# RajaeeKh/TriNerfLet

Measured on NVIDIA B200. Metric: rays/sec per training step (fwd+bwd), higher is better.
Workload: dtype f16

## Files before the change

include/trinerflet_b200.h:

```cpp
#ifndef TRINERFLET_B200_H
#define TRINERFLET_B200_H

#include <stdint.h>

#ifdef __cplusplus
extern "C" {
#endif

#define TNL_ABI_VERSION 1
#define TNL_ERR_INVALID_ARGUMENT (-1)
#define TNL_ERR_UNSUPPORTED (-2)
#define TNL_ERR_WORKSPACE (-3)

typedef void* tnl_stream_t;

int tnl_abi_version(void);
const char* tnl_last_error(void);

int tnl_near_far_from_aabb(const float* rays_o, const float* rays_d, const float* aabb, uint32_t N,
                           float min_near, float* nears, float* fars, tnl_stream_t stream);
int tnl_sph_from_ray(const float* rays_o, const float* rays_d, float radius, uint32_t N, float* coords,
                     tnl_stream_t stream);
int tnl_morton3d(const int32_t* coords, uint32_t N, int32_t* indices, tnl_stream_t stream);
int tnl_morton3d_invert(const int32_t* indices, uint32_t N, int32_t* coords, tnl_stream_t stream);
// ... 72 lines not shown
typedef struct tnl_mlp_dims {
    uint32_t in_dim;
    uint32_t hidden;
    uint32_t hidden_c;
} tnl_mlp_dims;
size_t tnl_mlp_packed_bytes(const tnl_mlp_dims* dims);
int tnl_mlp_pack_weights(const tnl_mlp_dims* dims, const float* W1, const float* W2, const float* W3,
                         const float* W4, const float* W5, void* packed, tnl_stream_t stream);
int tnl_mlp_forward(const tnl_mlp_dims* dims, const void* packed, const void* feat, int feat_fp16, const float* dirs,
                    uint32_t M, const int32_t* n_valid, float* sigma, float* rgb, float* geo,
                    tnl_stream_t stream);
int tnl_mlp_backward(const tnl_mlp_dims* dims, const void* packed, const void* feat, int feat_fp16, const float* dirs,
                     uint32_t M, const int32_t* n_valid, const float* g_sigma, const float* g_rgb,
                     void* g_feat, float* g_W1, float* g_W2, float* g_W3, float* g_W4, float* g_W5,
                     tnl_stream_t stream);

int tnl_umma_probe(const void* A, int a_rows, int a_cols, const void* B, int b_rows, int b_cols, int a_mn, int b_mn,
                   int M, int N, int K, float* out, int ncols, tnl_stream_t stream);

int tnl_umma_bench(int a_rows, int b_rows, int a_mn, int b_mn, int M, int N, int K, int reps, long long* out2,
                   tnl_stream_t stream);
int tnl_umma_bench2(uint32_t a_lbo, uint32_t a_sbo, uint32_t a_step, uint32_t a_type, uint32_t b_lbo, uint32_t b_sbo,
                    uint32_t b_step, uint32_t b_type, int a_mn, int b_mn, int M, int N, int ksteps, int reps, long long* out2,
                    tnl_stream_t stream);
int tnl_mlp_tc_profile(unsigned long long* counters64);

int tnl_grad_nonfinite(const float* g, uint64_t n, float* found_inf, tnl_stream_t stream);
int tnl_adam_prepare(float* state3, const float* found_inf, float beta1, float beta2, tnl_stream_t stream);
int tnl_adam_step(float* p, const float* g, float* m, float* v, uint64_t n, const float* inv_scale, const float* found_inf,
                  const float* state3, float lr, float beta1, float beta2, float eps, float weight_decay, tnl_stream_t stream);
// ... 33 lines not shown
```

trinerflet_b200/_lib.py:

```python
import ctypes
import os

import torch

_HERE = os.path.dirname(os.path.abspath(__file__))
LIB_PATH = os.path.join(_HERE, "lib", "libtrinerflet_b200.so")

_c = ctypes
_vp, _u32, _f32, _int, _sz = _c.c_void_p, _c.c_uint32, _c.c_float, _c.c_int, _c.c_size_t


class MlpDims(ctypes.Structure):
    _fields_ = [("in_dim", _u32), ("hidden", _u32), ("hidden_c", _u32)]


_DP = ctypes.POINTER(MlpDims)

SIGNATURES = {
    "tnl_abi_version": (_int, []),
    "tnl_last_error": (_c.c_char_p, []),
    "tnl_near_far_from_aabb": (_int, [_vp, _vp, _vp, _u32, _f32, _vp, _vp, _vp]),
    "tnl_sph_from_ray": (_int, [_vp, _vp, _f32, _u32, _vp, _vp]),
    "tnl_morton3d": (_int, [_vp, _u32, _vp, _vp]),
    "tnl_morton3d_invert": (_int, [_vp, _u32, _vp, _vp]),
# ... 14 lines not shown
    "tnl_composite_rays_dev": (_int, [_vp, _u32, _f32, _vp, _vp, _vp, _vp, _vp, _vp, _vp, _vp, _vp]),
    "tnl_compact_alive_dev": (_int, [_vp, _u32, _vp, _vp, _vp, _sz, _vp]),
    "tnl_sh_encode_forward": (_int, [_vp, _vp, _u32, _u32, _vp]),
    "tnl_idwt_level_forward": (_int, [_vp, _vp, _vp, _u32, _u32, _vp, _vp]),
    "tnl_idwt_level_backward": (_int, [_vp, _vp, _vp, _u32, _u32, _vp, _vp, _f32, _u32, _u32, _vp]),
    "tnl_sample_planes_forward": (_int, [_vp, _vp, _u32, _u32, _u32, _f32, _int, _vp, _vp, _vp, _int, _vp]),
    "tnl_sample_planes_backward": (_int, [_vp, _int, _vp, _u32, _u32, _u32, _f32, _int, _vp, _vp, _vp, _vp]),
    "tnl_sample_planes_backward_plane": (_int, [_vp, _int, _vp, _u32, _u32, _u32, _f32, _int, _vp, _vp, _vp, _u32, _vp]),
    "tnl_sample_planes_backward_coords": (_int, [_vp, _vp, _vp, _u32, _u32, _u32, _f32, _int, _vp, _vp]),
    "tnl_cell_sort_workspace": (_sz, [_u32, _u32]),
    "tnl_cell_sort": (_int, [_vp, _u32, _vp, _f32, _u32, _vp, _vp, _sz, _vp]),
    "tnl_mlp_packed_bytes": (_sz, [_DP]),
    "tnl_mlp_pack_weights": (_int, [_DP, _vp, _vp, _vp, _vp, _vp, _vp, _vp]),
    "tnl_mlp_forward": (_int, [_DP, _vp, _vp, _int, _vp, _u32, _vp, _vp, _vp, _vp, _vp]),
    "tnl_mlp_backward": (_int, [_DP, _vp, _vp, _int, _vp, _u32, _vp, _vp, _vp, _vp, _vp, _vp, _vp, _vp, _vp, _vp]),
    "tnl_idwt_level_forward_sparse": (_int, [_vp, _vp, _vp, _u32, _u32, _vp, _vp, _vp, _vp, _u32, _u32, _u32, _vp]),
    "tnl_idwt_level_backward_sparse": (_int, [_vp, _vp, _vp, _u32, _u32, _vp, _vp, _f32, _vp, _vp, _vp, _u32, _u32, _u32, _vp, _vp]),
    "tnl_tiles_zero": (_int, [_vp, _vp, _vp, _u32, _u32, _u32, _u32, _vp]),
    "tnl_mlp_tc_profile": (_int, [_vp]),
    "tnl_umma_bench": (_int, [_int] * 8 + [_vp, _vp]),
    "tnl_umma_bench2": (_int, [_u32] * 8 + [_int] * 6 + [_vp, _vp]),
    "tnl_umma_probe": (_int, [_vp, _int, _int, _vp, _int, _int, _int, _int, _int, _int, _int, _vp, _int, _vp]),
    "tnl_mark_dirty_tiles": (_int, [_vp, _u32, _u32, _f32, _u32, _u32, _u32, _vp, _vp]),
    "tnl_tiles_pack": (_int, [_vp, _vp, _u32, _u32, _u32, _u32, _vp, _int, _vp]),
    "tnl_tiles_unpack": (_int, [_vp, _vp, _u32, _u32, _u32, _u32, _f32, _int, _vp, _vp]),
    "tnl_tiles_allreduce": (_int, [_vp, _vp, _vp, _vp, _u32, _u32, _u32, _u32, _u32, _u32, _f32, _vp]),
    "tnl_flat_allreduce": (_int, [_vp, _vp, _u32, _u32, _u32, _f32, _vp]),
    "tnl_grad_nonfinite": (_int, [_vp, ctypes.c_uint64, _vp, _vp]),
    "tnl_adam_prepare": (_int, [_vp, _vp, _f32, _f32, _vp]),
    "tnl_adam_step": (_int, [_vp, _vp, _vp, _vp, ctypes.c_uint64, _vp, _vp, _vp, _f32, _f32, _f32, _f32, _f32, _vp]),
# ... 87 lines not shown
```

trinerflet_b200/csrc/mlp.cu:

```cuda
#include "common.cuh"
#include "mlp_math.cuh"
#include "mlp_tc.cuh"
#include <stdlib.h>

namespace tnl {

struct MlpLayout {
    int K1, H, HC;
    int F1, F2, F3, F4, F5;
    int B1, B2, B3, B4, B5;
    int total;
};

__host__ __device__ constexpr MlpLayout make_layout(int K1, int H, int HC) {
    MlpLayout L{};
    L.K1 = K1; L.H = H; L.HC = HC;
    L.F1 = 0;
    L.F2 = L.F1 + (K1 / 16) * (H / 8) * 64;
    L.F3 = L.F2 + (H / 16) * 2 * 64;
    L.F4 = L.F3 + 2 * (HC / 8) * 64;
    L.F5 = L.F4 + (HC / 16) * (HC / 8) * 64;
    L.B5 = L.F5 + (HC / 16) * 1 * 64;
    L.B4 = L.B5 + 1 * (HC / 8) * 64;
    L.B3 = L.B4 + (HC / 16) * (HC / 8) * 64;
// ... 547 lines not shown

static bool dims_supported(const tnl_mlp_dims* d) {
    if (!d) return false;
    const bool k_ok = d->in_dim == 48 || d->in_dim == 96 || d->in_dim == 144;
    const bool h_ok = (d->hidden == 64 && d->hidden_c == 64) || (d->hidden == 128 && d->hidden_c == 128);
    return k_ok && h_ok;
}

static size_t legacy_packed_bytes(const tnl_mlp_dims* d) {
    const size_t b = sizeof(uint32_t) * (size_t)make_layout((int)d->in_dim, (int)d->hidden, (int)d->hidden_c).total;
    return (b + 255) & ~(size_t)255;
}
static bool use_tc(const tnl_mlp_dims* d, int feat_fp16) {
    static const bool legacy = getenv("TNL_MLP_LEGACY") != nullptr;
    return !legacy && feat_fp16 && mlp_tc_supported(d->in_dim, d->hidden, d->hidden_c);
}

#define TNL_MLP_DISPATCH(DIMS, CALL)                                                        \
    do {                                                                                    \
        const uint32_t k_ = (DIMS)->in_dim, h_ = (DIMS)->hidden;                            \
        if (k_ == 48 && h_ == 64) { CALL(48, 64, 64); }                                     \
        else if (k_ == 96 && h_ == 64) { CALL(96, 64, 64); }                                \
        else if (k_ == 144 && h_ == 64) { CALL(144, 64, 64); }                              \
        else if (k_ == 48 && h_ == 128) { CALL(48, 128, 128); }                             \
        else if (k_ == 96 && h_ == 128) { CALL(96, 128, 128); }                             \
        else { CALL(144, 128, 128); }                                                       \
    } while (0)

extern "C" {

// ... 104 lines not shown
```

trinerflet_b200/csrc/mlp_tc.cu:

```cuda
#include "common.cuh"
#include "mlp_math.cuh"
#include "mlp_tc.cuh"
#include "mlp_tc_util.cuh"
#include "umma.cuh"
#include <stdlib.h>

namespace tnl {
using namespace umma;

template <int K1>
struct TcW {
    static constexpr uint32_t W1 = 0;
    static constexpr uint32_t W2 = W1 + tile_bytes(64, K1);
    static constexpr uint32_t W3 = W2 + tile_bytes(16, 64);
    static constexpr uint32_t W4 = W3 + tile_bytes(64, 32);
    static constexpr uint32_t W5 = W4 + tile_bytes(64, 64);
    static constexpr uint32_t END = W5 + tile_bytes(16, 64);
};

__global__ void k_mlp_tc_pack(int K1, int H, const float* __restrict__ W1, const float* __restrict__ W2, const float* __restrict__ W3,
                              const float* __restrict__ W4, const float* __restrict__ W5, uint8_t* __restrict__ out) {
    const uint32_t n1 = H * K1, n2 = 16 * H, n3 = H * 32, n4 = H * H, n5 = 16 * H;
    uint32_t i = blockIdx.x * blockDim.x + threadIdx.x;
    uint32_t base = 0, R, Cc;
// ... 154 lines not shown
    static constexpr uint32_t H4 = H3 + tile_bytes(128, 64);
    static constexpr uint32_t D5 = H4 + tile_bytes(128, 64);
    static constexpr uint32_t SUB = D5 + tile_bytes(128, 16);
    static constexpr uint32_t SUB0 = TcW<K1>::END;
    static constexpr uint32_t BAR = SUB0 + 2 * SUB;
    static constexpr uint32_t TOTAL = BAR + 48;
};

__device__ __forceinline__ bool m64_row_of_lane(uint32_t warp, uint32_t lane, uint32_t& row) {
    row = warp * 16 + lane;
    return lane < 16;
}

constexpr int kBwdStages = 10;

template <int K1>
__global__ void __launch_bounds__(544, 1)
k_mlp_tc_bwd(const uint8_t* __restrict__ wpk, const __half* __restrict__ feat, const float* __restrict__ dirs, uint32_t M,
             const int32_t* __restrict__ n_valid_ptr, const float* __restrict__ g_sigma, const float* __restrict__ g_rgb,
             __half* __restrict__ g_feat, float* __restrict__ gW1, float* __restrict__ gW2, float* __restrict__ gW3,
             float* __restrict__ gW4, float* __restrict__ gW5, unsigned long long* __restrict__ dbg) {
    using W = TcW<K1>;
    using S = TcBwdSmem<K1>;
    constexpr uint32_t CW = K1 < 64 ? 64 : K1;
    constexpr uint32_t TM_C = 0, TM_W1 = 2 * CW, TM_W4 = TM_W1 + K1, TM_W3 = TM_W4 + 64, TM_W2 = TM_W3 + 32, TM_W5 = TM_W2 + 16;
    constexpr uint32_t TM_COLS = 512;
    static_assert(TM_W5 + 16 <= TM_COLS, "TMEM column budget");
    extern __shared__ __align__(128) uint8_t smem[];
    const uint32_t tid = threadIdx.x, warp = tid >> 5, lane = tid & 31;
    uint64_t* ready = reinterpret_cast<uint64_t*>(smem + S::BAR);
    uint64_t* done = reinterpret_cast<uint64_t*>(smem + S::BAR + 16);
    uint32_t* tslot = reinterpret_cast<uint32_t*>(smem + S::BAR + 32);
    for (uint32_t i = tid * 16; i < W::END; i += 544 * 16) *reinterpret_cast<uint4*>(smem + i) = __ldg(reinterpret_cast<const uint4*>(wpk + i));
    if (tid == 0) {
        mbar_init(&ready[0], 256); mbar_init(&ready[1], 256);
        mbar_init(&done[0], 1); mbar_init(&done[1], 1);
// ... 92 lines not shown
        float a[32];                                                                                                    \
        tmem_load_row<32>(trow + hf * 32u, a);                                                                          \
        _Pragma("unroll") for (int kc = 0; kc < 4; ++kc)                                                                \
            *reinterpret_cast<uint4*>(sub + (TILE) + ((hf * 4u + kc) * 128u + t) * 16u) = pack8<true>(a + 8 * kc);     \
    }
#define TNL_EPI_MASK(TILE)                                                                                              \
    {                                                                                                                   \
        float a[32];                                                                                                    \
        tmem_load_row<32>(trow + hf * 32u, a);                                                                          \
        _Pragma("unroll") for (int kc = 0; kc < 4; ++kc) {                                                              \
            uint4* q = reinterpret_cast<uint4*>(sub + (TILE) + ((hf * 4u + kc) * 128u + t) * 16u);                      \
            *q = mask8(pack8<false>(a + 8 * kc), *q);                                                                   \
        }                                                                                                               \
    }
        uint4 x[XH];
        {
            const uint32_t p0 = (2 * blockIdx.x + g) * 128 + t;
            const uint4* src = reinterpret_cast<const uint4*>(feat + (size_t)p0 * K1) + hf * XH;
#pragma unroll
            for (int kc = 0; kc < XH; ++kc) x[kc] = (my_pairs > 0 && p0 < nvalid) ? __ldg(src + kc) : make_uint4(0u, 0u, 0u, 0u);
        }
        for (uint32_t it = 0; it < my_pairs; ++it) {
            const uint32_t tile = 2 * (blockIdx.x + it * gridDim.x) + g;
            const uint32_t p = tile * 128 + t;
            const bool v = p < nvalid;
#pragma unroll
            for (int kc = 0; kc < XH; ++kc) *reinterpret_cast<uint4*>(sub + S::X + ((hf * XH + kc) * 128 + t) * 16) = x[kc];
            float d[3] = {0.f, 0.f, 0.f}, gr[3] = {0.f, 0.f, 0.f}, gs = 0.f;
            if (v && hf == 0) {
#pragma unroll
                for (int j = 0; j < 3; ++j) { d[j] = __ldg(dirs + 3 * (size_t)p + j); gr[j] = __ldg(g_rgb + 3 * (size_t)p + j); }
                gs = __ldg(g_sigma + p);
            }
            TNL_HANDOFF();
            {
                const uint32_t pn = (2 * (blockIdx.x + (it + 1) * gridDim.x) + g) * 128 + t;
                const uint4* src = reinterpret_cast<const uint4*>(feat + (size_t)pn * K1) + hf * XH;
                const bool vn = (it + 1 < my_pairs) && pn < nvalid;
#pragma unroll
                for (int kc = 0; kc < XH; ++kc) x[kc] = vn ? __ldg(src + kc) : make_uint4(0u, 0u, 0u, 0u);
            }
            TNL_EPI_RELU(S::H1);
            TNL_HANDOFF();
            float logit = 0.f;
            if (hf == 0) {
                float h2[16];
                tmem_load_row<16>(trow, h2);
#pragma unroll
                for (int j = 0; j < 16; ++j) h2[j] = r16(h2[j]);
                logit = h2[0];
                float in3[32];
                {
                    float sh[16];
// ... 19 lines not shown
#pragma unroll
                for (int j = 0; j < 3; ++j) {
                    const float sg = r16(sigmoidf_(r16(o[j])));
                    d5[j] = v ? r16(gr[j]) * sg * (1.f - sg) : 0.f;
                }
#pragma unroll
                for (int j = 3; j < 8; ++j) d5[j] = 0.f;
                *reinterpret_cast<uint4*>(sub + S::D5 + (0 * 128 + t) * 16) = pack8<false>(d5);
                *reinterpret_cast<uint4*>(sub + S::D5 + (1 * 128 + t) * 16) = make_uint4(0u, 0u, 0u, 0u);
            }
            TNL_HANDOFF();
            TNL_EPI_MASK(S::H4);
            TNL_HANDOFF();
            TNL_EPI_MASK(S::H3);
            TNL_HANDOFF();
            if (hf == 0) {
                float a[16];
                tmem_load_row<16>(trow, a);
                float dh2[16];
                dh2[0] = gs * expf(fminf(fmaxf(logit, -15.f), 15.f));
#pragma unroll
                for (int j = 0; j < 15; ++j) dh2[1 + j] = a[j];
                *reinterpret_cast<uint4*>(sub + S::I3 + (0 * 128 + t) * 16) = pack8<false>(dh2);
                *reinterpret_cast<uint4*>(sub + S::I3 + (1 * 128 + t) * 16) = pack8<false>(dh2 + 8);
            }
            TNL_HANDOFF();
            TNL_EPI_MASK(S::H1);
            TNL_HANDOFF();
            {
                float a[KH];
                tmem_load_row<KH>(trow + hf * KH, a);
                if (g_feat && p < M) {
                    uint4* dst = reinterpret_cast<uint4*>(g_feat + (size_t)p * K1 + hf * KH);
#pragma unroll
                    for (int kc = 0; kc < KH / 8; ++kc) dst[kc] = v ? pack8<false>(a + 8 * kc) : make_uint4(0u, 0u, 0u, 0u);
                }
            }
        }
#undef TNL_HANDOFF
#undef TNL_EPI_RELU
#undef TNL_EPI_MASK
    }
    fence_before_sync();
    __syncthreads();
// ... 185 lines not shown
                                                              n_valid, sigma, rgb, geo);
    else
        k_mlp_tc_fwd<K1, false><<<blocks, 128, S::TOTAL, s>>>(static_cast<const uint8_t*>(wpk), static_cast<const __half*>(feat), dirs, M,
                                                               n_valid, sigma, rgb, geo);
}

void mlp_tc_forward(uint32_t in_dim, uint32_t hidden, const void* wpk, const void* feat, const float* dirs, uint32_t M,
                    const int32_t* n_valid, float* sigma, float* rgb, float* geo, cudaStream_t s) {
    if (hidden == 128) { mlp_tc128_forward(in_dim, wpk, feat, dirs, M, n_valid, sigma, rgb, geo, s); return; }
    if (in_dim == 48) launch_fwd<48>(wpk, feat, dirs, M, n_valid, sigma, rgb, geo, s);
    else launch_fwd<96>(wpk, feat, dirs, M, n_valid, sigma, rgb, geo, s);
}

static unsigned long long* g_tc_dbg = nullptr;

template <int K1>
static void launch_bwd(const void* wpk, const void* feat, const float* dirs, uint32_t M, const int32_t* n_valid, const float* g_sigma,
                       const float* g_rgb, void* g_feat, float* gW1, float* gW2, float* gW3, float* gW4, float* gW5, cudaStream_t s) {
    using S = TcBwdSmem<K1>;
    cudaFuncSetAttribute(k_mlp_tc_bwd<K1>, cudaFuncAttributeMaxDynamicSharedMemorySize, (int)S::TOTAL);
    const uint32_t blocks = min(ceil_div(M, 256u), (uint32_t)kNumSM);
    k_mlp_tc_bwd<K1><<<blocks, 544, S::TOTAL, s>>>(static_cast<const uint8_t*>(wpk), static_cast<const __half*>(feat), dirs, M, n_valid,
                                                   g_sigma, g_rgb, static_cast<__half*>(g_feat), gW1, gW2, gW3, gW4, gW5, g_tc_dbg);
}

void mlp_tc_backward(uint32_t in_dim, uint32_t hidden, const void* wpk, const void* feat, const float* dirs, uint32_t M,
                     const int32_t* n_valid, const float* g_sigma, const float* g_rgb, void* g_feat, float* gW1, float* gW2, float* gW3,
                     float* gW4, float* gW5, cudaStream_t s) {
    if (hidden == 128) { mlp_tc128_backward(in_dim, wpk, feat, dirs, M, n_valid, g_sigma, g_rgb, g_feat, gW1, gW2, gW3, gW4, gW5, s); return; }
    if (in_dim == 48) launch_bwd<48>(wpk, feat, dirs, M, n_valid, g_sigma, g_rgb, g_feat, gW1, gW2, gW3, gW4, gW5, s);
    else launch_bwd<96>(wpk, feat, dirs, M, n_valid, g_sigma, g_rgb, g_feat, gW1, gW2, gW3, gW4, gW5, s);
}

}

using namespace tnl;

extern "C" int tnl_mlp_tc_profile(unsigned long long* counters64) {
    g_tc_dbg = counters64;
    return 0;
}

extern "C" int tnl_umma_bench(int a_rows, int b_rows, int a_mn, int b_mn, int M, int N, int K, int reps, long long* out2,
                              tnl_stream_t stream) {
    TNL_ARG_CHECK(out2, "null pointer");
    static bool attr = false;
    if (!attr) {
        cudaFuncSetAttribute(k_umma_bench, cudaFuncAttributeMaxDynamicSharedMemorySize, 160 * 1024);
        attr = true;
    }
    k_umma_bench<<<1, 128, 160 * 1024, reinterpret_cast<cudaStream_t>(stream)>>>(a_rows, b_rows, a_mn, b_mn, M, N, K, reps, out2);
    return finish_launch("umma_bench");
}

extern "C" int tnl_umma_bench2(uint32_t a_lbo, uint32_t a_sbo, uint32_t a_step, uint32_t a_type, uint32_t b_lbo, uint32_t b_sbo,
// ... 31 lines not shown
```

trinerflet_b200/csrc/mlp_tc.cuh:

```cuda
#pragma once
#include <cuda_runtime.h>
#include <stddef.h>
#include <stdint.h>

namespace tnl {

bool mlp_tc_supported(uint32_t in_dim, uint32_t hidden, uint32_t hidden_c);
size_t mlp_tc_packed_bytes(uint32_t in_dim, uint32_t hidden);
void mlp_tc_pack(uint32_t in_dim, uint32_t hidden, const float* W1, const float* W2, const float* W3, const float* W4, const float* W5,
                 void* out, cudaStream_t s);
void mlp_tc_forward(uint32_t in_dim, uint32_t hidden, const void* wpk, const void* feat, const float* dirs, uint32_t M,
                    const int32_t* n_valid, float* sigma, float* rgb, float* geo, cudaStream_t s);
void mlp_tc_backward(uint32_t in_dim, uint32_t hidden, const void* wpk, const void* feat, const float* dirs, uint32_t M,
                     const int32_t* n_valid, const float* g_sigma, const float* g_rgb, void* g_feat, float* gW1, float* gW2, float* gW3,
                     float* gW4, float* gW5, cudaStream_t s);
void mlp_tc128_forward(uint32_t in_dim, const void* wpk, const void* feat, const float* dirs, uint32_t M, const int32_t* n_valid,
                       float* sigma, float* rgb, float* geo, cudaStream_t s);
void mlp_tc128_backward(uint32_t in_dim, const void* wpk, const void* feat, const float* dirs, uint32_t M, const int32_t* n_valid,
                        const float* g_sigma, const float* g_rgb, void* g_feat, float* gW1, float* gW2, float* gW3, float* gW4, float* gW5,
                        cudaStream_t s);

}
```

trinerflet_b200/csrc/sample_coords.cuh:

```cuda
#pragma once
#include "common.cuh"

namespace tnl {

struct Tap {
    int x0, y0;
    float nw, ne, sw, se;
    bool x1ok, y1ok;
};

__device__ __forceinline__ float to_pixel(float g, int R) {
    float v = ((g + 1.0f) * 0.5f) * (float)(R - 1);
    return fminf((float)(R - 1), fmaxf(v, 0.0f));
}

__device__ __forceinline__ float to_pixel_grad(float g, int R, float& dg) {
    const float hi = (float)(R - 1);
    const float v = ((g + 1.0f) * 0.5f) * hi;
    if (!(v > 0.0f)) { dg = 0.0f; return 0.0f; }
    if (v >= hi) { dg = 0.0f; return hi; }
    dg = 0.5f * hi;
    return v;
}

// ... 1 lines not shown
    const float ix = to_pixel(gx, R), iy = to_pixel(gy, R);
    const float fx = floorf(ix), fy = floorf(iy);
    Tap t;
    t.x0 = (int)fx;
    t.y0 = (int)fy;
    const float ex = fx + 1.0f, ey = fy + 1.0f;
    t.nw = (ex - ix) * (ey - iy);
    t.ne = (ix - fx) * (ey - iy);
    t.sw = (ex - ix) * (iy - fy);
    t.se = (ix - fx) * (iy - fy);
    t.x1ok = t.x0 + 1 <= R - 1;
    t.y1ok = t.y0 + 1 <= R - 1;
    return t;
}

__device__ __forceinline__ float axis_coord(const float* __restrict__ xyz, uint32_t m, int a, float inv_bound, int fp16_coords) {
    float g = __fmul_rn(__ldg(xyz + 3 * (size_t)m + a), inv_bound);
    if (fp16_coords) g = __half2float(__float2half_rn(g));
    return g;
}

__device__ __forceinline__ void plane_coords(const float* __restrict__ xyz, uint32_t m, int p, float inv_bound,
                                             int fp16_coords, float& gx, float& gy) {
    const int a = (p == 2) ? 1 : 0;
    const int b = (p == 1) ? 1 : 2;
    gx = axis_coord(xyz, m, a, inv_bound, fp16_coords);
    gy = axis_coord(xyz, m, b, inv_bound, fp16_coords);
}

__device__ __forceinline__ uint2 pack4h(float4 v) {
    const __half2 a = __floats2half2_rn(v.x, v.y), b = __floats2half2_rn(v.z, v.w);
    return make_uint2(*reinterpret_cast<const uint32_t*>(&a), *reinterpret_cast<const uint32_t*>(&b));
}
__device__ __forceinline__ float4 unpack4h(uint2 u) {
// ... 6 lines not shown
```

trinerflet_b200/network.py:

```python
import ctypes

import torch
import torch.nn as nn
import torch.nn.functional as F
from torch.autograd import Function

from . import _lib
from ._lib import MlpDims, call, ptr, stream
from .activation import trunc_exp
from .encoding import get_encoder
from .renderer import NeRFRenderer


def fused_dims_supported(in_dim, hidden, hidden_color):
    return in_dim in (48, 96, 144) and hidden == hidden_color and hidden in (64, 128)


def pack_mlp_weights(dims, weights):
    lib = _lib.load()
    nbytes = lib.tnl_mlp_packed_bytes(ctypes.byref(dims))
    if nbytes == 0:
        raise RuntimeError("trinerflet_b200: unsupported MLP dimensions for the fused kernel")
    packed = torch.empty(nbytes, dtype=torch.uint8, device=weights[0].device)
    ws = [w.detach().contiguous().float() for w in weights]
    call("tnl_mlp_pack_weights", ctypes.byref(dims), *[ptr(w) for w in ws], ptr(packed), stream())
    return packed
# ... 1 lines not shown

_warned_library_path = False


def _warn_library_path(net, x):
    global _warned_library_path
    if not _warned_library_path and x.is_cuda:
        import warnings
        why = ("MLP dimensions outside the fused kernels" if not fused_dims_supported(net.in_dim, net.hidden_dim, net.hidden_dim_color)
               else "no CUDA fp16 autocast is active")
        warnings.warn(f"trinerflet_b200.NeRFNetwork: {why}; the sigma/color heads run as plain torch ops (library GEMMs), not the "
                      "fused sm_100a kernels. Wrap the call in torch.autocast('cuda', dtype=torch.float16) as the reference's --fp16 does.")
        _warned_library_path = True


class _FieldMLP(Function):

    @staticmethod
    def forward(ctx, feat, dirs, n_valid, W1, W2, W3, W4, W5):
        feat = feat.contiguous()
        ctx.in_dtype = feat.dtype
        if W1.shape[0] != 64:
            feat = feat.half()
        elif feat.dtype != torch.float16:
            feat = feat.float()
        fh = int(feat.dtype == torch.float16)
        dirs = dirs.detach().contiguous().float()
        M = feat.shape[0]
        dims = MlpDims(W1.shape[1], W1.shape[0], W4.shape[0])
        packed = pack_mlp_weights(dims, (W1, W2, W3, W4, W5))
        sigma = torch.empty(M, device=feat.device, dtype=torch.float32)
        rgb = torch.empty(M, 3, device=feat.device, dtype=torch.float32)
        call("tnl_mlp_forward", ctypes.byref(dims), ptr(packed), ptr(feat), fh, ptr(dirs), M, ptr(n_valid), ptr(sigma),
             ptr(rgb), None, stream())
        ctx.save_for_backward(feat, dirs, packed, n_valid if n_valid is not None else torch.empty(0))
        ctx.dims = (dims.in_dim, dims.hidden, dims.hidden_c, n_valid is not None)
        ctx.wshapes = [tuple(w.shape) for w in (W1, W2, W3, W4, W5)]
        return sigma, rgb

    @staticmethod
    def backward(ctx, g_sigma, g_rgb):
        feat, dirs, packed, n_valid = ctx.saved_tensors
        in_dim, hidden, hidden_c, has_nv = ctx.dims
        dims = MlpDims(in_dim, hidden, hidden_c)
        M = feat.shape[0]
        g_sigma = g_sigma.contiguous().float()
        g_rgb = g_rgb.contiguous().float()
        g_feat = torch.empty_like(feat)
        gW = [torch.zeros(s, device=feat.device, dtype=torch.float32) for s in ctx.wshapes]
        call("tnl_mlp_backward", ctypes.byref(dims), ptr(packed), ptr(feat), int(feat.dtype == torch.float16), ptr(dirs), M,
             ptr(n_valid) if has_nv else None, ptr(g_sigma), ptr(g_rgb), ptr(g_feat), *[ptr(g) for g in gW], stream())
        if g_feat.dtype != ctx.in_dtype:
            g_feat = g_feat.to(ctx.in_dtype)
        return (g_feat, None, None, *gW)


class _DensityMLP(Function):

    @staticmethod
    def forward(ctx, feat, W1, W2, W3, W4, W5):
        feat = feat.contiguous()
        if feat.dtype != torch.float16:
            feat = feat.float()
        M = feat.shape[0]
        dims = MlpDims(W1.shape[1], W1.shape[0], W4.shape[0])
        packed = pack_mlp_weights(dims, (W1, W2, W3, W4, W5))
        sigma = torch.empty(M, device=feat.device, dtype=torch.float32)
        geo = torch.empty(M, 15, device=feat.device, dtype=torch.float32)
        call("tnl_mlp_forward", ctypes.byref(dims), ptr(packed), ptr(feat), int(feat.dtype == torch.float16), None, M, None,
# ... 36 lines not shown
        return (self.sigma_net[0].weight, self.sigma_net[1].weight, self.color_net[0].weight, self.color_net[1].weight,
                self.color_net[2].weight)

    def _fused(self):
        return (torch.is_autocast_enabled("cuda") and torch.get_autocast_dtype("cuda") == torch.float16
                and fused_dims_supported(self.in_dim, self.hidden_dim, self.hidden_dim_color))

    spatial_sort_min_points = 1 << 18

    def forward(self, x, d, n_valid=None):
        perm = None
        if x.is_cuda and x.shape[0] >= self.spatial_sort_min_points and torch.is_grad_enabled():
            from .triplane_encoder import cell_sort
            perm = cell_sort(x, self.bound, n_valid, 64)
        fused = self._fused()
        feat = self.encoder(x, bound=self.bound, n_valid=n_valid, perm=perm, half_out=fused)
        if fused:
            return _FieldMLP.apply(feat, d, n_valid, *self._weights())
        _warn_library_path(self, x)
        h = F.relu(self.sigma_net[0](feat))
        h = self.sigma_net[1](h)
        sigma = trunc_exp(h[..., 0])
        geo_feat = h[..., 1:]
        h = torch.cat([self.encoder_dir(d), geo_feat], dim=-1)
        h = F.relu(self.color_net[0](h))
        h = F.relu(self.color_net[1](h))
        color = torch.sigmoid(self.color_net[2](h))
        return sigma, color

    def density(self, x):
# ... 31 lines not shown
```

trinerflet_b200/triplane_encoder.py:

```python
import math

import numpy as np
import torch
import torch.nn as nn
from torch.autograd import Function

from ._lib import call, ptr, stream

PAD_DICT = {'bior6.8': 4}


def get_levels(upscale_factor):
    wavelet_levels = math.log2(upscale_factor)
    if abs(wavelet_levels - round(wavelet_levels)) > 1e-5:
        raise ValueError('Unsupported res. should be 2^')
    return round(wavelet_levels)


def cl_empty_planes(C, n, device=None, dtype=torch.float32, zero=False):
    f = torch.zeros if zero else torch.empty
    return f(3, n, n, C, device=device, dtype=dtype).permute(0, 3, 1, 2)


def cl_empty_coefs(C, n, device=None, dtype=torch.float32, zero=False):
# ... 166 lines not shown
            p.grad = g


def build_planes_with_abs(planes_features, coefs, plan=None):
    return _BuildPlanes.apply(planes_features, plan, *coefs)


def build_planes(planes_features, coefs, plan=None):
    return _BuildPlanes.apply(planes_features, plan, *coefs)[0]


def _inv_bound(bound):
    return float(np.float32(1.0) / np.float32(bound))


class _SamplePlanes(Function):
    @staticmethod
    def forward(ctx, planes, coords, bound, fp16_coords, n_valid, perm=None, half_out=False, grad_buf=None):
        _require_cuda_f32(planes, "planes")
        ctx.grad_buf = grad_buf
        planes_cl = to_cl_planes(planes.detach())
        coords = coords.detach().contiguous().float()
        M = coords.shape[0]
        C, R = planes.shape[1], planes.shape[2]
        feat = torch.empty(M, 3 * C, device=planes.device, dtype=torch.float16 if half_out else torch.float32)
        inv = _inv_bound(bound)
        call("tnl_sample_planes_forward", ptr(planes_cl), ptr(coords), M, R, C, inv, int(bool(fp16_coords)),
             ptr(n_valid), ptr(perm), ptr(feat), int(bool(half_out)), stream())
        ctx.save_for_backward(coords, n_valid if n_valid is not None else torch.empty(0),
                              perm if perm is not None else torch.empty(0))
        ctx.meta = (M, R, C, inv, int(bool(fp16_coords)), n_valid is not None, perm is not None, bool(half_out))
        return feat

    @staticmethod
    def backward(ctx, g_feat):
        coords, n_valid, perm = ctx.saved_tensors
        M, R, C, inv, fp16_coords, has_nv, has_perm, half = ctx.meta
        g_feat = g_feat.contiguous().half() if half else g_feat.contiguous().float()
        external = False
        if ctx.grad_buf is not None:
            g_planes, ready, external, plane_hook = ctx.grad_buf
            ctx.grad_buf = None
            torch.cuda.current_stream().wait_event(ready)
        else:
            g_planes = cl_empty_planes(C, R, device=g_feat.device, zero=True)
            plane_hook = None
        if plane_hook is not None and C in (16, 32, 48):
            for p in range(3):
                call("tnl_sample_planes_backward_plane", ptr(g_feat), int(half), ptr(coords), M, R, C, inv, fp16_coords,
                     ptr(n_valid) if has_nv else None, ptr(perm) if has_perm else None, ptr(g_planes), p, stream())
                plane_hook(p)
        else:
            call("tnl_sample_planes_backward", ptr(g_feat), int(half), ptr(coords), M, R, C, inv, fp16_coords,
                 ptr(n_valid) if has_nv else None, ptr(perm) if has_perm else None, ptr(g_planes), stream())
        if external:
            return None, None, None, None, None, None, None, None
        return g_planes, None, None, None, None, None, None, None


def cell_sort(coords, bound, n_valid=None, G=64):
    from . import _lib
# ... 222 lines not shown
    def get_grid_features(self, grid_res, plane_features=None, grid=None):
        if grid is None:
            axis = torch.arange(grid_res)
            gx, gy, gz = torch.meshgrid(axis, axis, axis, indexing='xy')
            grid = torch.stack([gx, gy, gz], dim=-1) / (grid_res - 1)
        assert grid.max() <= 1 and grid.min() >= 0
        grid = 2 * self.lbound * grid - self.lbound
        grid = grid[..., [2, 0, 1]]
        if plane_features is None:
            plane_features = self.get_planes(2 * grid_res)
        grid = grid.to(device=plane_features.device, dtype=plane_features.dtype)
        shape = grid.shape
        feats = self.sample_from_planes(grid.reshape(-1, 3), plane_features=plane_features)
        return self.lbound, feats.reshape(*shape[:-1], -1), grid

    def forward(self, coordinates, bound, n_valid=None, perm=None, half_out=False):
        planes = self.get_planes()
        gbuf = self._join_prefetch()
        if gbuf is not None and not torch.is_grad_enabled():
            gbuf = None
        return sample_planes(planes, coordinates, bound, n_valid=n_valid, perm=perm, half_out=half_out, grad_buf=gbuf)

    def _load_from_state_dict(self, state_dict, prefix, *args, **kwargs):
        super()._load_from_state_dict(state_dict, prefix, *args, **kwargs)
        self.last_used_planes = None
```

Baseline: 11.54 million.

## Fuse triplane gradient scatter into tcgen05 MLP backward kernel

Adds a SCATTER variant of the tcgen05 MLP backward kernel. Instead of writing g_feat to global memory and running a separate sample-planes backward kernel, it stages the input-feature gradient in shared memory and scatters it with bilinear weights into the plane gradients using vector red.add atomics. A new autograd Function fuses plane sampling and the MLP for the 64-wide heads when a cell-sort permutation exists, reading rows through perm. This removes the g_feat round trip and one kernel launch. The cost is more register and shared-memory pressure and atomic work inside the pipelined MLP kernel, which could stall its tensor-core stages.

```diff
diff --git a/include/trinerflet_b200.h b/include/trinerflet_b200.h
--- a/include/trinerflet_b200.h
+++ b/include/trinerflet_b200.h
@@ -110,6 +110,10 @@
                      uint32_t M, const int32_t* n_valid, const float* g_sigma, const float* g_rgb,
                      void* g_feat, float* g_W1, float* g_W2, float* g_W3, float* g_W4, float* g_W5,
                      tnl_stream_t stream);
+int tnl_mlp_backward_scatter(const tnl_mlp_dims* dims, const void* packed, const void* feat, const float* dirs, uint32_t M,
+                             const int32_t* n_valid, const int32_t* perm, const float* g_sigma, const float* g_rgb,
+                             const float* xyz, uint32_t R, uint32_t C, float inv_bound, int fp16_coords, float* g_planes,
+                             float* g_W1, float* g_W2, float* g_W3, float* g_W4, float* g_W5, tnl_stream_t stream);
 
 int tnl_umma_probe(const void* A, int a_rows, int a_cols, const void* B, int b_rows, int b_cols, int a_mn, int b_mn,
                    int M, int N, int K, float* out, int ncols, tnl_stream_t stream);
diff --git a/profiles/prof_bwd_kernels.py b/profiles/prof_bwd_kernels.py
--- /dev/null
+++ b/profiles/prof_bwd_kernels.py
@@ -0,0 +1,41 @@
+import json
+import os
+import sys
+
+sys.path.insert(0, os.path.dirname(os.path.dirname(os.path.abspath(__file__))))
+import torch
+from torch.profiler import ProfilerActivity, profile
+
+from trinerflet_b200 import scene, trainer
+from trinerflet_b200.network import NeRFNetwork
+
+name = os.environ.get("TNL_CONFIG", "base_light")
+cfg = scene.CONFIGS[name]
+steps = int(os.environ.get("TNL_STEPS", "10"))
+net = NeRFNetwork(bound=1.5, cuda_ray=True, density_thresh=10, min_near=0.2, triplane_channels=cfg["C"],
+                  triplane_resolution=cfg["R"], triplane_wavelet_levels=cfg["S"], hidden_dim=cfg["hidden"],
+                  hidden_dim_color=cfg["hidden"]).cuda()
+scene.init_model_(net, 0)
+scene.install_ball_occupancy(net, 0.75)
+ts = trainer.TrainStep(net, trainer.default_opt(), None)
+sc = scene.make_scene()
+g = torch.Generator().manual_seed(0)
+batches = [tuple(t.cuda() for t in scene.sample_batch(sc, cfg["rays"], g)) for _ in range(steps + 3)]
+ts.forward_backward(*batches[0], update_grid=False)
+net.mean_count = int(net.step_counter[0, 0].item())
+net.local_step = 0
+for b in batches[1:3]:
+    net.zero_grad(set_to_none=True)
+    ts.forward_backward(*b, update_grid=False)
+torch.cuda.synchronize()
+with profile(activities=[ProfilerActivity.CUDA]) as prof:
+    for b in batches[3:]:
+        net.zero_grad(set_to_none=True)
+        ts.forward_backward(*b, update_grid=False)
+    torch.cuda.synchronize()
+per = {}
+for ev in prof.key_averages():
+    if "k_mlp_tc_bwd" in ev.key or "k_sample_bwd4" in ev.key:
+        per[ev.key] = round(ev.device_time_total / 1e3 / steps, 4)
+print(json.dumps({"config": name, "samples": net.mean_count, "steps": steps, "device": torch.cuda.get_device_name(0),
+                  "ms_per_step": per, "sum_ms_per_step": round(sum(per.values()), 4)}))
diff --git a/trinerflet_b200/_lib.py b/trinerflet_b200/_lib.py
--- a/trinerflet_b200/_lib.py
+++ b/trinerflet_b200/_lib.py
@@ -52,6 +52,8 @@
     "tnl_mlp_pack_weights": (_int, [_DP, _vp, _vp, _vp, _vp, _vp, _vp, _vp]),
     "tnl_mlp_forward": (_int, [_DP, _vp, _vp, _int, _vp, _u32, _vp, _vp, _vp, _vp, _vp]),
     "tnl_mlp_backward": (_int, [_DP, _vp, _vp, _int, _vp, _u32, _vp, _vp, _vp, _vp, _vp, _vp, _vp, _vp, _vp, _vp]),
+    "tnl_mlp_backward_scatter": (_int, [_DP, _vp, _vp, _vp, _u32, _vp, _vp, _vp, _vp, _vp, _u32, _u32, _f32, _int, _vp, _vp, _vp,
+                                        _vp, _vp, _vp, _vp]),
     "tnl_idwt_level_forward_sparse": (_int, [_vp, _vp, _vp, _u32, _u32, _vp, _vp, _vp, _vp, _u32, _u32, _u32, _vp]),
     "tnl_idwt_level_backward_sparse": (_int, [_vp, _vp, _vp, _u32, _u32, _vp, _vp, _f32, _vp, _vp, _vp, _u32, _u32, _u32, _vp, _vp]),
     "tnl_tiles_zero": (_int, [_vp, _vp, _vp, _u32, _u32, _u32, _u32, _vp]),
diff --git a/trinerflet_b200/csrc/mlp.cu b/trinerflet_b200/csrc/mlp.cu
--- a/trinerflet_b200/csrc/mlp.cu
+++ b/trinerflet_b200/csrc/mlp.cu
@@ -585,6 +585,11 @@
 static bool use_tc(const tnl_mlp_dims* d, int feat_fp16) {
     static const bool legacy = getenv("TNL_MLP_LEGACY") != nullptr;
     return !legacy && feat_fp16 && mlp_tc_supported(d->in_dim, d->hidden, d->hidden_c);
+}
+
+namespace tnl {
+size_t mlp_tc_packed_offset(const tnl_mlp_dims* d) { return legacy_packed_bytes(d); }
+bool mlp_tc_selected(const tnl_mlp_dims* d) { return dims_supported(d) && use_tc(d, 1); }
 }
 
 #define TNL_MLP_DISPATCH(DIMS, CALL)                                                        \
diff --git a/trinerflet_b200/csrc/mlp_tc.cu b/trinerflet_b200/csrc/mlp_tc.cu
--- a/trinerflet_b200/csrc/mlp_tc.cu
+++ b/trinerflet_b200/csrc/mlp_tc.cu
@@ -2,6 +2,7 @@
 #include "mlp_math.cuh"
 #include "mlp_tc.cuh"
 #include "mlp_tc_util.cuh"
+#include "sample_coords.cuh"
 #include "umma.cuh"
 #include <stdlib.h>
 
@@ -192,12 +193,27 @@
 
 constexpr int kBwdStages = 10;
 
-template <int K1>
+struct PlaneScatter {
+    const int32_t* perm;
+    const float* xyz;
+    float* g_planes;
+    int R;
+    float inv_bound;
+    int fp16_coords;
+};
+
+__device__ __forceinline__ void red_add_v4(float* addr, float4 v, float w) {
+    asm volatile("red.global.add.v4.f32 [%0], {%1, %2, %3, %4};\n" ::"l"(addr), "f"(v.x * w), "f"(v.y * w), "f"(v.z * w),
+                 "f"(v.w * w)
+                 : "memory");
+}
+
+template <int K1, bool SCATTER>
 __global__ void __launch_bounds__(544, 1)
 k_mlp_tc_bwd(const uint8_t* __restrict__ wpk, const __half* __restrict__ feat, const float* __restrict__ dirs, uint32_t M,
              const int32_t* __restrict__ n_valid_ptr, const float* __restrict__ g_sigma, const float* __restrict__ g_rgb,
              __half* __restrict__ g_feat, float* __restrict__ gW1, float* __restrict__ gW2, float* __restrict__ gW3,
-             float* __restrict__ gW4, float* __restrict__ gW5, unsigned long long* __restrict__ dbg) {
+             float* __restrict__ gW4, float* __restrict__ gW5, unsigned long long* __restrict__ dbg, const PlaneScatter sc) {
     using W = TcW<K1>;
     using S = TcBwdSmem<K1>;
     constexpr uint32_t CW = K1 < 64 ? 64 : K1;
@@ -320,29 +336,34 @@
         }                                                                                                               \
     }
         uint4 x[XH];
+        uint32_t mx;
         {
             const uint32_t p0 = (2 * blockIdx.x + g) * 128 + t;
-            const uint4* src = reinterpret_cast<const uint4*>(feat + (size_t)p0 * K1) + hf * XH;
-#pragma unroll
-            for (int kc = 0; kc < XH; ++kc) x[kc] = (my_pairs > 0 && p0 < nvalid) ? __ldg(src + kc) : make_uint4(0u, 0u, 0u, 0u);
+            const bool v0 = my_pairs > 0 && p0 < nvalid;
+            mx = (SCATTER && v0) ? (uint32_t)__ldg(sc.perm + p0) : p0;
+            const uint4* src = reinterpret_cast<const uint4*>(feat + (size_t)mx * K1) + hf * XH;
+#pragma unroll
+            for (int kc = 0; kc < XH; ++kc) x[kc] = v0 ? __ldg(src + kc) : make_uint4(0u, 0u, 0u, 0u);
         }
         for (uint32_t it = 0; it < my_pairs; ++it) {
             const uint32_t tile = 2 * (blockIdx.x + it * gridDim.x) + g;
             const uint32_t p = tile * 128 + t;
             const bool v = p < nvalid;
+            const uint32_t m = mx;
 #pragma unroll
             for (int kc = 0; kc < XH; ++kc) *reinterpret_cast<uint4*>(sub + S::X + ((hf * XH + kc) * 128 + t) * 16) = x[kc];
             float d[3] = {0.f, 0.f, 0.f}, gr[3] = {0.f, 0.f, 0.f}, gs = 0.f;
             if (v && hf == 0) {
 #pragma unroll
-                for (int j = 0; j < 3; ++j) { d[j] = __ldg(dirs + 3 * (size_t)p + j); gr[j] = __ldg(g_rgb + 3 * (size_t)p + j); }
-                gs = __ldg(g_sigma + p);
+                for (int j = 0; j < 3; ++j) { d[j] = __ldg(dirs + 3 * (size_t)m + j); gr[j] = __ldg(g_rgb + 3 * (size_t)m + j); }
+                gs = __ldg(g_sigma + m);
             }
             TNL_HANDOFF();
             {
                 const uint32_t pn = (2 * (blockIdx.x + (it + 1) * gridDim.x) + g) * 128 + t;
-                const uint4* src = reinterpret_cast<const uint4*>(feat + (size_t)pn * K1) + hf * XH;
                 const bool vn = (it + 1 < my_pairs) && pn < nvalid;
+                mx = (SCATTER && vn) ? (uint32_t)__ldg(sc.perm + pn) : pn;
+                const uint4* src = reinterpret_cast<const uint4*>(feat + (size_t)mx * K1) + hf * XH;
 #pragma unroll
                 for (int kc = 0; kc < XH; ++kc) x[kc] = vn ? __ldg(src + kc) : make_uint4(0u, 0u, 0u, 0u);
             }
@@ -392,6 +413,11 @@
             TNL_HANDOFF();
             TNL_EPI_MASK(S::H3);
             TNL_HANDOFF();
+            float pos[3] = {0.f, 0.f, 0.f};
+            if (SCATTER && v) {
+#pragma unroll
+                for (int j = 0; j < 3; ++j) pos[j] = __ldg(sc.xyz + 3 * (size_t)m + j);
+            }
             if (hf == 0) {
                 float a[16];
                 tmem_load_row<16>(trow, a);
@@ -405,7 +431,43 @@
             TNL_HANDOFF();
             TNL_EPI_MASK(S::H1);
             TNL_HANDOFF();
-            {
+            if constexpr (SCATTER) {
+                constexpr int C = K1 / 3, CH = KH % 16 == 0 ? 16 : 8, RS = 2 * K1 + 16;
+                static_assert(128 * RS + 128 * 12 <= 2 * tile_bytes(128, 64), "staging area exceeds the H3 | H4 tiles");
+                uint8_t* stg = sub + S::H3;
+                float* su = reinterpret_cast<float*>(stg + 128 * RS);
+#pragma unroll
+                for (int j = 0; j < KH / CH; ++j) {
+                    float a[CH];
+                    tmem_load_row<CH>(trow + hf * KH + j * CH, a);
+#pragma unroll
+                    for (int kc = 0; kc < CH / 8; ++kc)
+                        *reinterpret_cast<uint4*>(stg + t * RS + (hf * KH + j * CH + 8 * kc) * 2) = pack8<false>(a + 8 * kc);
+                }
+                if (hf == 0) {
+#pragma unroll
+                    for (int j = 0; j < 3; ++j) su[3 * t + j] = project_coord(pos[j], sc.inv_bound, sc.fp16_coords);
+                }
+                asm volatile("bar.sync %0, 256;" ::"r"(1u + g) : "memory");
+                const uint32_t r = hf * 128 + t;
+                const uint32_t nvt = nvalid - tile * 128 < 128u ? nvalid - tile * 128 : 128u;
+#pragma unroll 4
+                for (int k = 0; k < K1 / 8; ++k) {
+                    const uint32_t task = k * 256 + r;
+                    const uint32_t q = task % (C / 4), pl = (task / (C / 4)) % 3, pt = task / (3 * C / 4);
+                    if (pt >= nvt) break;
+                    const float4 gq = unpack4h(*reinterpret_cast<const uint2*>(stg + pt * RS + (pl * C + 4 * q) * 2));
+                    if (gq.x == 0.f && gq.y == 0.f && gq.z == 0.f && gq.w == 0.f) continue;
+                    const float* u = su + 3 * pt;
+                    const Tap tp = make_tap(pl == 2 ? u[1] : u[0], pl == 1 ? u[1] : u[2], sc.R);
+                    float* base = sc.g_planes + (((size_t)pl * sc.R + tp.y0) * sc.R + tp.x0) * C + 4 * q;
+                    const size_t dx = (size_t)C, dy = (size_t)sc.R * C;
+                    red_add_v4(base, gq, tp.nw);
+                    if (tp.x1ok) red_add_v4(base + dx, gq, tp.ne);
+                    if (tp.y1ok) red_add_v4(base + dy, gq, tp.sw);
+                    if (tp.x1ok && tp.y1ok) red_add_v4(base + dy + dx, gq, tp.se);
+                }
+            } else {
                 float a[KH];
                 tmem_load_row<KH>(trow + hf * KH, a);
                 if (g_feat && p < M) {
@@ -621,22 +683,25 @@
 
 static unsigned long long* g_tc_dbg = nullptr;
 
-template <int K1>
+template <int K1, bool SCATTER>
 static void launch_bwd(const void* wpk, const void* feat, const float* dirs, uint32_t M, const int32_t* n_valid, const float* g_sigma,
-                       const float* g_rgb, void* g_feat, float* gW1, float* gW2, float* gW3, float* gW4, float* gW5, cudaStream_t s) {
+                       const float* g_rgb, void* g_feat, float* gW1, float* gW2, float* gW3, float* gW4, float* gW5, const PlaneScatter& sc,
+                       cudaStream_t s) {
     using S = TcBwdSmem<K1>;
-    cudaFuncSetAttribute(k_mlp_tc_bwd<K1>, cudaFuncAttributeMaxDynamicSharedMemorySize, (int)S::TOTAL);
+    cudaFuncSetAttribute(k_mlp_tc_bwd<K1, SCATTER>, cudaFuncAttributeMaxDynamicSharedMemorySize, (int)S::TOTAL);
     const uint32_t blocks = min(ceil_div(M, 256u), (uint32_t)kNumSM);
-    k_mlp_tc_bwd<K1><<<blocks, 544, S::TOTAL, s>>>(static_cast<const uint8_t*>(wpk), static_cast<const __half*>(feat), dirs, M, n_valid,
-                                                   g_sigma, g_rgb, static_cast<__half*>(g_feat), gW1, gW2, gW3, gW4, gW5, g_tc_dbg);
+    k_mlp_tc_bwd<K1, SCATTER><<<blocks, 544, S::TOTAL, s>>>(static_cast<const uint8_t*>(wpk), static_cast<const __half*>(feat), dirs, M,
+                                                            n_valid, g_sigma, g_rgb, static_cast<__half*>(g_feat), gW1, gW2, gW3, gW4,
+                                                            gW5, g_tc_dbg, sc);
 }
 
 void mlp_tc_backward(uint32_t in_dim, uint32_t hidden, const void* wpk, const void* feat, const float* dirs, uint32_t M,
                      const int32_t* n_valid, const float* g_sigma, const float* g_rgb, void* g_feat, float* gW1, float* gW2, float* gW3,
                      float* gW4, float* gW5, cudaStream_t s) {
     if (hidden == 128) { mlp_tc128_backward(in_dim, wpk, feat, dirs, M, n_valid, g_sigma, g_rgb, g_feat, gW1, gW2, gW3, gW4, gW5, s); return; }
-    if (in_dim == 48) launch_bwd<48>(wpk, feat, dirs, M, n_valid, g_sigma, g_rgb, g_feat, gW1, gW2, gW3, gW4, gW5, s);
-    else launch_bwd<96>(wpk, feat, dirs, M, n_valid, g_sigma, g_rgb, g_feat, gW1, gW2, gW3, gW4, gW5, s);
+    const PlaneScatter none{};
+    if (in_dim == 48) launch_bwd<48, false>(wpk, feat, dirs, M, n_valid, g_sigma, g_rgb, g_feat, gW1, gW2, gW3, gW4, gW5, none, s);
+    else launch_bwd<96, false>(wpk, feat, dirs, M, n_valid, g_sigma, g_rgb, g_feat, gW1, gW2, gW3, gW4, gW5, none, s);
 }
 
 }
@@ -646,6 +711,27 @@
 extern "C" int tnl_mlp_tc_profile(unsigned long long* counters64) {
     g_tc_dbg = counters64;
     return 0;
+}
+
+extern "C" int tnl_mlp_backward_scatter(const tnl_mlp_dims* dims, const void* packed, const void* feat, const float* dirs, uint32_t M,
+                                        const int32_t* n_valid, const int32_t* perm, const float* g_sigma, const float* g_rgb,
+                                        const float* xyz, uint32_t R, uint32_t C, float inv_bound, int fp16_coords, float* g_planes,
+                                        float* g_W1, float* g_W2, float* g_W3, float* g_W4, float* g_W5, tnl_stream_t stream) {
+    if (M == 0) return 0;
+    if (!dims || !mlp_tc_selected(dims) || dims->hidden != 64 || dims->in_dim != 3 * C) {
+        set_error("mlp_backward_scatter: the 64-wide heads on the tcgen05 kernels (in_dim = 3C in {48, 96}, hidden = hidden_color = 64)");
+        return TNL_ERR_UNSUPPORTED;
+    }
+    TNL_ARG_CHECK(packed && feat && dirs && perm && g_sigma && g_rgb && xyz && g_planes && g_W1 && g_W2 && g_W3 && g_W4 && g_W5,
+                  "null pointer");
+    TNL_ARG_CHECK(R >= 2, "R >= 2");
+    TNL_ARG_CHECK(((uintptr_t)feat & 15) == 0 && ((uintptr_t)g_planes & 15) == 0, "feat/g_planes must be 16-byte aligned");
+    const PlaneScatter sc{perm, xyz, g_planes, (int)R, inv_bound, fp16_coords};
+    const uint8_t* wpk = static_cast<const uint8_t*>(packed) + mlp_tc_packed_offset(dims);
+    cudaStream_t s = reinterpret_cast<cudaStream_t>(stream);
+    if (C == 16) launch_bwd<48, true>(wpk, feat, dirs, M, n_valid, g_sigma, g_rgb, nullptr, g_W1, g_W2, g_W3, g_W4, g_W5, sc, s);
+    else launch_bwd<96, true>(wpk, feat, dirs, M, n_valid, g_sigma, g_rgb, nullptr, g_W1, g_W2, g_W3, g_W4, g_W5, sc, s);
+    return finish_launch("mlp_backward_scatter(tcgen05)");
 }
 
 extern "C" int tnl_umma_bench(int a_rows, int b_rows, int a_mn, int b_mn, int M, int N, int K, int reps, long long* out2,
diff --git a/trinerflet_b200/csrc/mlp_tc.cuh b/trinerflet_b200/csrc/mlp_tc.cuh
--- a/trinerflet_b200/csrc/mlp_tc.cuh
+++ b/trinerflet_b200/csrc/mlp_tc.cuh
@@ -1,6 +1,7 @@
 #pragma once
 #include <cuda_runtime.h>
 #include <stddef.h>
+#include "../../include/trinerflet_b200.h"
 #include <stdint.h>
 
 namespace tnl {
@@ -14,6 +15,8 @@
 void mlp_tc_backward(uint32_t in_dim, uint32_t hidden, const void* wpk, const void* feat, const float* dirs, uint32_t M,
                      const int32_t* n_valid, const float* g_sigma, const float* g_rgb, void* g_feat, float* gW1, float* gW2, float* gW3,
                      float* gW4, float* gW5, cudaStream_t s);
+size_t mlp_tc_packed_offset(const tnl_mlp_dims* dims);
+bool mlp_tc_selected(const tnl_mlp_dims* dims);
 void mlp_tc128_forward(uint32_t in_dim, const void* wpk, const void* feat, const float* dirs, uint32_t M, const int32_t* n_valid,
                        float* sigma, float* rgb, float* geo, cudaStream_t s);
 void mlp_tc128_backward(uint32_t in_dim, const void* wpk, const void* feat, const float* dirs, uint32_t M, const int32_t* n_valid,
diff --git a/trinerflet_b200/csrc/sample_coords.cuh b/trinerflet_b200/csrc/sample_coords.cuh
--- a/trinerflet_b200/csrc/sample_coords.cuh
+++ b/trinerflet_b200/csrc/sample_coords.cuh
@@ -39,10 +39,14 @@
     return t;
 }
 
-__device__ __forceinline__ float axis_coord(const float* __restrict__ xyz, uint32_t m, int a, float inv_bound, int fp16_coords) {
-    float g = __fmul_rn(__ldg(xyz + 3 * (size_t)m + a), inv_bound);
+__device__ __forceinline__ float project_coord(float x, float inv_bound, int fp16_coords) {
+    float g = __fmul_rn(x, inv_bound);
     if (fp16_coords) g = __half2float(__float2half_rn(g));
     return g;
+}
+
+__device__ __forceinline__ float axis_coord(const float* __restrict__ xyz, uint32_t m, int a, float inv_bound, int fp16_coords) {
+    return project_coord(__ldg(xyz + 3 * (size_t)m + a), inv_bound, fp16_coords);
 }
 
 __device__ __forceinline__ void plane_coords(const float* __restrict__ xyz, uint32_t m, int p, float inv_bound,
diff --git a/trinerflet_b200/network.py b/trinerflet_b200/network.py
--- a/trinerflet_b200/network.py
+++ b/trinerflet_b200/network.py
@@ -10,6 +10,7 @@
 from .activation import trunc_exp
 from .encoding import get_encoder
 from .renderer import NeRFRenderer
+from .triplane_encoder import gather_features, take_grad_buffer
 
 
 def fused_dims_supported(in_dim, hidden, hidden_color):
@@ -41,6 +42,18 @@
         _warned_library_path = True
 
 
+def _mlp_forward(feat, dirs, n_valid, W):
+    dirs = dirs.detach().contiguous().float()
+    M = feat.shape[0]
+    dims = MlpDims(W[0].shape[1], W[0].shape[0], W[3].shape[0])
+    packed = pack_mlp_weights(dims, W)
+    sigma = torch.empty(M, device=feat.device, dtype=torch.float32)
+    rgb = torch.empty(M, 3, device=feat.device, dtype=torch.float32)
+    call("tnl_mlp_forward", ctypes.byref(dims), ptr(packed), ptr(feat), int(feat.dtype == torch.float16), ptr(dirs), M, ptr(n_valid),
+         ptr(sigma), ptr(rgb), None, stream())
+    return sigma, rgb, dirs, packed, dims
+
+
 class _FieldMLP(Function):
 
     @staticmethod
@@ -51,15 +64,7 @@
             feat = feat.half()
         elif feat.dtype != torch.float16:
             feat = feat.float()
-        fh = int(feat.dtype == torch.float16)
-        dirs = dirs.detach().contiguous().float()
-        M = feat.shape[0]
-        dims = MlpDims(W1.shape[1], W1.shape[0], W4.shape[0])
-        packed = pack_mlp_weights(dims, (W1, W2, W3, W4, W5))
-        sigma = torch.empty(M, device=feat.device, dtype=torch.float32)
-        rgb = torch.empty(M, 3, device=feat.device, dtype=torch.float32)
-        call("tnl_mlp_forward", ctypes.byref(dims), ptr(packed), ptr(feat), fh, ptr(dirs), M, ptr(n_valid), ptr(sigma),
-             ptr(rgb), None, stream())
+        sigma, rgb, dirs, packed, dims = _mlp_forward(feat, dirs, n_valid, (W1, W2, W3, W4, W5))
         ctx.save_for_backward(feat, dirs, packed, n_valid if n_valid is not None else torch.empty(0))
         ctx.dims = (dims.in_dim, dims.hidden, dims.hidden_c, n_valid is not None)
         ctx.wshapes = [tuple(w.shape) for w in (W1, W2, W3, W4, W5)]
@@ -80,6 +85,33 @@
         if g_feat.dtype != ctx.in_dtype:
             g_feat = g_feat.to(ctx.in_dtype)
         return (g_feat, None, None, *gW)
+
+
+class _Field(Function):
+
+    @staticmethod
+    def forward(ctx, planes, coords, dirs, bound, n_valid, perm, grad_buf, W1, W2, W3, W4, W5):
+        ctx.grad_buf = grad_buf
+        feat, coords, ctx.meta = gather_features(planes, coords, bound, True, n_valid, perm, True)
+        sigma, rgb, dirs, packed, dims = _mlp_forward(feat, dirs, n_valid, (W1, W2, W3, W4, W5))
+        ctx.save_for_backward(feat, coords, dirs, packed, n_valid if n_valid is not None else torch.empty(0), perm)
+        ctx.dims = (dims.in_dim, dims.hidden, dims.hidden_c)
+        ctx.wshapes = [tuple(w.shape) for w in (W1, W2, W3, W4, W5)]
+        return sigma, rgb
+
+    @staticmethod
+    def backward(ctx, g_sigma, g_rgb):
+        feat, coords, dirs, packed, n_valid, perm = ctx.saved_tensors
+        M, R, C, inv, fp16_coords, has_nv, _, _ = ctx.meta
+        dims = MlpDims(*ctx.dims)
+        g_planes, external, plane_hook = take_grad_buffer(ctx, C, R, feat.device)
+        assert plane_hook is None, "the plane-by-plane exchange scatters through _SamplePlanes"
+        g_sigma = g_sigma.contiguous().float()
+        g_rgb = g_rgb.contiguous().float()
+        gW = [torch.zeros(s, device=feat.device, dtype=torch.float32) for s in ctx.wshapes]
+        call("tnl_mlp_backward_scatter", ctypes.byref(dims), ptr(packed), ptr(feat), ptr(dirs), M, ptr(n_valid) if has_nv else None,
+             ptr(perm), ptr(g_sigma), ptr(g_rgb), ptr(coords), R, C, inv, fp16_coords, ptr(g_planes), *[ptr(g) for g in gW], stream())
+        return (None if external else g_planes, None, None, None, None, None, None, *gW)
 
 
 class _DensityMLP(Function):
@@ -146,6 +178,10 @@
             from .triplane_encoder import cell_sort
             perm = cell_sort(x, self.bound, n_valid, 64)
         fused = self._fused()
+        if (fused and perm is not None and self.hidden_dim == 64 and self.in_dim in (48, 96)
+                and self.encoder.scatter_plane_hook is None):
+            planes, gbuf = self.encoder.planes_and_grad_buffer()
+            return _Field.apply(planes, x, d, self.bound, n_valid, perm, gbuf, *self._weights())
         feat = self.encoder(x, bound=self.bound, n_valid=n_valid, perm=perm, half_out=fused)
         if fused:
             return _FieldMLP.apply(feat, d, n_valid, *self._weights())
diff --git a/trinerflet_b200/triplane_encoder.py b/trinerflet_b200/triplane_encoder.py
--- a/trinerflet_b200/triplane_encoder.py
+++ b/trinerflet_b200/triplane_encoder.py
@@ -204,22 +204,35 @@
     return float(np.float32(1.0) / np.float32(bound))
 
 
+def gather_features(planes, coords, bound, fp16_coords, n_valid, perm, half_out):
+    _require_cuda_f32(planes, "planes")
+    planes_cl = to_cl_planes(planes.detach())
+    coords = coords.detach().contiguous().float()
+    M = coords.shape[0]
+    C, R = planes.shape[1], planes.shape[2]
+    feat = torch.empty(M, 3 * C, device=planes.device, dtype=torch.float16 if half_out else torch.float32)
+    inv = _inv_bound(bound)
+    call("tnl_sample_planes_forward", ptr(planes_cl), ptr(coords), M, R, C, inv, int(bool(fp16_coords)),
+         ptr(n_valid), ptr(perm), ptr(feat), int(bool(half_out)), stream())
+    return feat, coords, (M, R, C, inv, int(bool(fp16_coords)), n_valid is not None, perm is not None, bool(half_out))
+
+
+def take_grad_buffer(ctx, C, R, device):
+    if ctx.grad_buf is None:
+        return cl_empty_planes(C, R, device=device, zero=True), False, None
+    g_planes, ready, external, plane_hook = ctx.grad_buf
+    ctx.grad_buf = None
+    torch.cuda.current_stream().wait_event(ready)
+    return g_planes, external, plane_hook
+
+
 class _SamplePlanes(Function):
     @staticmethod
     def forward(ctx, planes, coords, bound, fp16_coords, n_valid, perm=None, half_out=False, grad_buf=None):
-        _require_cuda_f32(planes, "planes")
         ctx.grad_buf = grad_buf
-        planes_cl = to_cl_planes(planes.detach())
-        coords = coords.detach().contiguous().float()
-        M = coords.shape[0]
-        C, R = planes.shape[1], planes.shape[2]
-        feat = torch.empty(M, 3 * C, device=planes.device, dtype=torch.float16 if half_out else torch.float32)
-        inv = _inv_bound(bound)
-        call("tnl_sample_planes_forward", ptr(planes_cl), ptr(coords), M, R, C, inv, int(bool(fp16_coords)),
-             ptr(n_valid), ptr(perm), ptr(feat), int(bool(half_out)), stream())
+        feat, coords, ctx.meta = gather_features(planes, coords, bound, fp16_coords, n_valid, perm, half_out)
         ctx.save_for_backward(coords, n_valid if n_valid is not None else torch.empty(0),
                               perm if perm is not None else torch.empty(0))
-        ctx.meta = (M, R, C, inv, int(bool(fp16_coords)), n_valid is not None, perm is not None, bool(half_out))
         return feat
 
     @staticmethod
@@ -227,14 +240,7 @@
         coords, n_valid, perm = ctx.saved_tensors
         M, R, C, inv, fp16_coords, has_nv, has_perm, half = ctx.meta
         g_feat = g_feat.contiguous().half() if half else g_feat.contiguous().float()
-        external = False
-        if ctx.grad_buf is not None:
-            g_planes, ready, external, plane_hook = ctx.grad_buf
-            ctx.grad_buf = None
-            torch.cuda.current_stream().wait_event(ready)
-        else:
-            g_planes = cl_empty_planes(C, R, device=g_feat.device, zero=True)
-            plane_hook = None
+        g_planes, external, plane_hook = take_grad_buffer(ctx, C, R, g_feat.device)
         if plane_hook is not None and C in (16, 32, 48):
             for p in range(3):
                 call("tnl_sample_planes_backward_plane", ptr(g_feat), int(half), ptr(coords), M, R, C, inv, fp16_coords,
@@ -487,11 +493,15 @@
         feats = self.sample_from_planes(grid.reshape(-1, 3), plane_features=plane_features)
         return self.lbound, feats.reshape(*shape[:-1], -1), grid
 
-    def forward(self, coordinates, bound, n_valid=None, perm=None, half_out=False):
+    def planes_and_grad_buffer(self):
         planes = self.get_planes()
         gbuf = self._join_prefetch()
         if gbuf is not None and not torch.is_grad_enabled():
             gbuf = None
+        return planes, gbuf
+
+    def forward(self, coordinates, bound, n_valid=None, perm=None, half_out=False):
+        planes, gbuf = self.planes_and_grad_buffer()
         return sample_planes(planes, coordinates, bound, n_valid=n_valid, perm=perm, half_out=half_out, grad_buf=gbuf)
 
     def _load_from_state_dict(self, state_dict, prefix, *args, **kwargs):
```

Result: faster. 11.93 million (median of 6 runs) (+3.4%).
